# aristoteleo/spateo-release

Hardware: AMD Instinct MI355X
Metric: cells/s per SparseVFC EM iter (higher is better)
Workload: dtype f32

## Files before the change

### spateo-release_amd/csrc/mvf_common.h

```cpp
#pragma once
#include <hip/hip_runtime.h>

#include <cmath>
#include <cstdarg>
#include <cstdint>
#include <cstdio>
#include <cstdlib>
#include <algorithm>

#include "../../include/mvf.h"

namespace mvf {

char* err_buf();
int set_error(const char* fmt, ...);
enum DebugOpt { DBG_CONK_FORM = 0, DBG_SLICE_LEN, DBG_SOLVE_SMALL_OFF, DBG_LR_TIMING, DBG_LR_NO_DEFLATE, DBG_DEFL_BLOCK, DBG_DEFL_APPS, DBG_LR_NO_DIRECT, DBG_DIRECT_ACCEPT, DBG_COUNT };
long long debug_opt(DebugOpt which);
int device_cu_count();

#define MVF_CHECK_HIP(expr)                                                                      \
    do {                                                                                         \
        hipError_t _e = (expr);                                                                  \
        if (_e != hipSuccess) return ::mvf::set_error("%s failed: %s", #expr, hipGetErrorString(_e)); \
    } while (0)

#define MVF_REQUIRE(cond, ...)                       \
    do {                                             \
        if (!(cond)) return ::mvf::set_error(__VA_ARGS__); \
    } while (0)

#define MVF_LAUNCH_CHECK() MVF_CHECK_HIP(hipGetLastError())

constexpr int WAVE = 64;

constexpr double LOG2E = 1.4426950408889634074;

template <typename T>
struct Vec4;
template <>
struct Vec4<float> {
    using type = float4;
};
template <>
struct Vec4<double> {
    using type = double4;
};

__device__ __forceinline__ float exp2_neg(float e) { return __builtin_amdgcn_exp2f(e); }
__device__ __forceinline__ double exp2_neg(double e) { return exp2(e); }

template <typename T>
__device__ __forceinline__ T kernel_value(T px, T py, T pz, T cx, T cy, T cz) {
    const T dx = px - cx, dy = py - cy, dz = pz - cz;
    const T e = fma(dz, dz, fma(dy, dy, dx * dx));
    return exp2_neg(-e);
}

template <int D, typename T>
__device__ __forceinline__ T kernel_value_d(const T (&p)[D], const T (&c)[D]) {
    T e = T(0);
#pragma unroll
    for (int k = 0; k < D; ++k) {
        const T t = p[k] - c[k];
        e = fma(t, t, e);
    }
    return exp2_neg(-e);
}

__device__ __forceinline__ double wave_sum(double v) {
#pragma unroll
    for (int o = 32; o > 0; o >>= 1) v += __shfl_down(v, o, 64);
    return v;
}
__device__ __forceinline__ double wave_min(double v) {
#pragma unroll
    for (int o = 32; o > 0; o >>= 1) v = fmin(v, __shfl_down(v, o, 64));
    return v;
}

template <int NT>
__device__ __forceinline__ double block_sum(double v, double* sm ) {
    v = wave_sum(v);
    const int lane = threadIdx.x & 63, w = threadIdx.x >> 6;
    __syncthreads();
    if (lane == 0) sm[w] = v;
    __syncthreads();
    double t = 0.0;
    if (threadIdx.x == 0) {
#pragma unroll
        for (int i = 0; i < NT / 64; ++i) t += sm[i];
    }
    return t;
}
template <int NT>
__device__ __forceinline__ double block_min(double v, double* sm) {
    v = wave_min(v);
    const int lane = threadIdx.x & 63, w = threadIdx.x >> 6;
    __syncthreads();
    if (lane == 0) sm[w] = v;
    __syncthreads();
    double t = INFINITY;
    if (threadIdx.x == 0) {
#pragma unroll
        for (int i = 0; i < NT / 64; ++i) t = fmin(t, sm[i]);
    }
    return t;
}

struct EvalAffine {
    double alpha[3], jmul;
    double A[9];
    double b[3];
};

inline EvalAffine eval_affine_from_host(const double* affine) {
    EvalAffine af;
    af.alpha[0] = af.alpha[1] = af.alpha[2] = 1.0, af.jmul = 1.0;
    for (int i = 0; i < 9; ++i) af.A[i] = 0.0;
    for (int i = 0; i < 3; ++i) af.b[i] = 0.0;
    if (affine) {
        for (int i = 0; i < 3; ++i) af.alpha[i] = affine[i];
        af.jmul = affine[3];
        for (int i = 0; i < 9; ++i) af.A[i] = affine[4 + i];
        for (int i = 0; i < 3; ++i) af.b[i] = affine[13 + i];
    }
    return af;
}

inline int64_t cdiv(int64_t a, int64_t b) { return (a + b - 1) / b; }
inline size_t align_up(size_t x, size_t a) { return (x + a - 1) / a * a; }

}
```

### spateo-release_amd/csrc/mvf_em.hip

```cpp
#include "mvf_common.h"

namespace mvf {

constexpr int APPLY_CHUNK = 512;

template <typename T, int CPT>
__global__ __launch_bounds__(256) void apply_kernel(const T* __restrict__ x4, int64_t n, const T* __restrict__ ctrl4,
                                                    int64_t m, T s, const double* __restrict__ C ,
                                                    T* __restrict__ V4, const T* __restrict__ y4,
                                                    const T* __restrict__ P, T* __restrict__ r,
                                                    double* __restrict__ block_pr) {
    using V4T = typename Vec4<T>::type;
    __shared__ __attribute__((aligned(16))) unsigned char smem_raw[APPLY_CHUNK * (sizeof(V4T) + 4 * sizeof(double))];
    V4T* sc = reinterpret_cast<V4T*>(smem_raw);
    double4* sC = reinterpret_cast<double4*>(smem_raw + APPLY_CHUNK * sizeof(V4T));

    const int64_t base = ((int64_t)blockIdx.x * 256) * CPT + threadIdx.x;
    T px[CPT], py[CPT], pz[CPT];
    double v0[CPT], v1[CPT], v2[CPT];
#pragma unroll
    for (int c = 0; c < CPT; ++c) {
        const int64_t i = base + (int64_t)c * 256;
        V4T xv = (i < n) ? reinterpret_cast<const V4T*>(x4)[i] : V4T{0, 0, 0, 0};
        px[c] = xv.x * s;
        py[c] = xv.y * s;
        pz[c] = xv.z * s;
        v0[c] = v1[c] = v2[c] = 0.0;
    }

    for (int64_t m0 = 0; m0 < m; m0 += APPLY_CHUNK) {
        const int mc = (int)min((int64_t)APPLY_CHUNK, m - m0);
        __syncthreads();
        for (int j = threadIdx.x; j < APPLY_CHUNK; j += 256) {
            if (j < mc) {
                V4T cv = reinterpret_cast<const V4T*>(ctrl4)[m0 + j];
                sc[j] = V4T{cv.x * s, cv.y * s, cv.z * s, 0};
                const double* cp = C + (m0 + j) * 3;
                sC[j] = double4{cp[0], cp[1], cp[2], 0.0};
            } else {
                sc[j] = V4T{0, 0, 0, 0};
                sC[j] = double4{0.0, 0.0, 0.0, 0.0};
            }
        }
        __syncthreads();
        const int mc_pad = (mc + 3) & ~3;
#pragma unroll 4
        for (int j = 0; j < mc_pad; ++j) {
            const V4T cv = sc[j];
            const double4 cc = sC[j];
#pragma unroll
            for (int c = 0; c < CPT; ++c) {
                const double k = (double)kernel_value(px[c], py[c], pz[c], cv.x, cv.y, cv.z);
                v0[c] = fma(k, cc.x, v0[c]);
                v1[c] = fma(k, cc.y, v1[c]);
                v2[c] = fma(k, cc.z, v2[c]);
            }
        }
    }

    double pr = 0.0;
#pragma unroll
    for (int c = 0; c < CPT; ++c) {
        const int64_t i = base + (int64_t)c * 256;
        if (i < n) {
            reinterpret_cast<V4T*>(V4)[i] = V4T{(T)v0[c], (T)v1[c], (T)v2[c], 0};
            if (y4) {
                const V4T yv = reinterpret_cast<const V4T*>(y4)[i];
                const double d0 = (double)yv.x - (double)(T)v0[c], d1 = (double)yv.y - (double)(T)v1[c],
                             d2 = (double)yv.z - (double)(T)v2[c];
                const double rr = d0 * d0 + d1 * d1 + d2 * d2;
                r[i] = (T)rr;
                if (P) pr += (double)P[i] * (double)(T)rr;
            }
        }
    }
    if (y4 && P && block_pr) {
        __shared__ double red[4];
        const double t = block_sum<256>(pr, red);
        if (threadIdx.x == 0) block_pr[blockIdx.x] = t;
    }
}

__global__ __launch_bounds__(256) void sum_partials_kernel(const double* __restrict__ partials, int64_t nb, int stride,
                                                           int K, double* __restrict__ out, int overwrite = 0) {
    __shared__ double red[4];
    for (int k = 0; k < K; ++k) {
        double s = 0.0;
        for (int64_t b = threadIdx.x; b < nb; b += 256) s += partials[b * stride + k];
        const double t = block_sum<256>(s, red);
        if (threadIdx.x == 0) out[k] = overwrite ? t : out[k] + t;
        __syncthreads();
    }
}

template <typename T>
__global__ __launch_bounds__(256) void estep_min_kernel(const T* __restrict__ r, int64_t n, double inv2s2,
                                                        double* __restrict__ block_min_out,
                                                        double* __restrict__ block_zero_out) {
    double mn = INFINITY, zeros = 0.0;
    for (int64_t i = (int64_t)blockIdx.x * 256 + threadIdx.x; i < n; i += (int64_t)gridDim.x * 256) {
        const double t1 = exp(-(double)r[i] * inv2s2);
        if (t1 == 0.0)
            zeros += 1.0;
        else
            mn = fmin(mn, t1);
    }
    __shared__ double red[4];
    const double bm = block_min<256>(mn, red);
    const double bz = block_sum<256>(zeros, red);
    if (threadIdx.x == 0) {
        block_min_out[blockIdx.x] = bm;
        block_zero_out[blockIdx.x] = bz;
    }
}

__global__ __launch_bounds__(256) void estep_min_finish(const double* __restrict__ bmin, const double* __restrict__ bzero,
                                                        int nb, double* __restrict__ mins) {
    double mn = INFINITY, z = 0.0;
    for (int i = threadIdx.x; i < nb; i += 256) {
        mn = fmin(mn, bmin[i]);
        z += bzero[i];
    }
    __shared__ double red[4];
    const double a = block_min<256>(mn, red);
    const double b = block_sum<256>(z, red);
    if (threadIdx.x == 0) {
        mins[0] = a;
        mins[1] = b;
    }
}

template <typename T>
__global__ __launch_bounds__(256) void estep_p_kernel(const T* __restrict__ r, int64_t n, double inv2s2, double t2,
                                                      double minP, double theta, double zero_fill_host,
                                                      const double* __restrict__ fill_dev, T* __restrict__ Pout,
                                                      double* __restrict__ block_stats) {
    double zero_fill = zero_fill_host;
    if (fill_dev) {
        const double f = *fill_dev;
        zero_fill = (f < INFINITY) ? f : 0.0;
    }
    double s_pr = 0.0, s_p = 0.0, s_pf = 0.0, s_cnt = 0.0, s_zero = 0.0;
    for (int64_t i = (int64_t)blockIdx.x * 256 + threadIdx.x; i < n; i += (int64_t)gridDim.x * 256) {
        const double ri = (double)r[i];
        double t1 = exp(-ri * inv2s2);
        if (t1 == 0.0) {
            t1 = zero_fill;
            s_zero += 1.0;
        }
        const double p = t1 / (t1 + t2);
        s_pr += p * ri;
        s_p += p;
        const T pf = (T)fmax(p, minP);
        Pout[i] = pf;
        s_pf += (double)pf;
        s_cnt += ((double)pf > theta) ? 1.0 : 0.0;
    }
    __shared__ double red[4];
    const double a = block_sum<256>(s_pr, red);
    const double b = block_sum<256>(s_p, red);
    const double c = block_sum<256>(s_pf, red);
    const double d = block_sum<256>(s_cnt, red);
    const double e = block_sum<256>(s_zero, red);
    if (threadIdx.x == 0) {
        double* o = block_stats + (int64_t)blockIdx.x * 5;
        o[0] = a, o[1] = b, o[2] = c, o[3] = d, o[4] = e;
    }
}

__global__ __launch_bounds__(256) void quadform_kernel(const double* __restrict__ K, const double* __restrict__ C,
                                                       int64_t m, int nrhs, double* __restrict__ row_out) {
    const int64_t i = blockIdx.x;
    double acc = 0.0;
    for (int d = 0; d < nrhs; ++d) {
        double t = 0.0;
        for (int64_t j = threadIdx.x; j < m; j += 256) t += K[i * m + j] * C[j * nrhs + d];
        acc += t * C[i * nrhs + d];
    }
    __shared__ double red[4];
    const double s = block_sum<256>(acc, red);
    if (threadIdx.x == 0) row_out[i] = s;
}

__device__ __forceinline__ int64_t tri_offset(int64_t i, int64_t m) { return i * m - i * (i - 1) / 2; }

__global__ __launch_bounds__(256) void sym_pack_kernel(const double* __restrict__ G, int64_t m, double* __restrict__ tri) {
    const int64_t i = blockIdx.y;
    const int64_t j = (int64_t)blockIdx.x * 256 + threadIdx.x;
    if (j < m && j >= i) tri[tri_offset(i, m) + (j - i)] = G[i * m + j];
}

__global__ __launch_bounds__(256) void sym_unpack_kernel(const double* __restrict__ tri, int64_t m, double* __restrict__ G) {
    const int64_t i = blockIdx.y;
    const int64_t j = (int64_t)blockIdx.x * 256 + threadIdx.x;
    if (j >= m) return;
    G[i * m + j] = j >= i ? tri[tri_offset(i, m) + (j - i)] : tri[tri_offset(j, m) + (i - j)];
}

}

using namespace mvf;

extern "C" int mvf_sym_pack(const double* G, int64_t m, double* tri, void* stream) {
    MVF_REQUIRE(m >= 0 && m <= 65535, "mvf_sym_pack: bad m");
    if (m == 0) return 0;
// ... 167 lines not shown
```

### spateo-release_amd/csrc/mvf_gram.hip

```cpp
#include "mvf_common.h"
#include <type_traits>

namespace mvf {

constexpr int GT = 128;
constexpr int GCHUNK = 256;

typedef double f64x4 __attribute__((ext_vector_type(4)));

struct GramPlan {
    int nt = 0, npairs = 0;
    int njobs = 0, edge2 = 0;
    int64_t slice_len = 0, nslices = 0;
    int64_t phase_slices = 0, nphases = 1;
    int64_t rslice_len = 0, rslices = 0;
    int rcolblocks = 0;
    size_t gram_bytes = 0, rhs_bytes = 0;
};

constexpr int RHS_CPT = 2;
constexpr int RHS_COLS = 256 * RHS_CPT;

static int gram_slots() { return 2 * device_cu_count(); }

// ... 88 lines not shown
        const int64_t ib = (int64_t)tj * GT + wj * 64 + a * 16 + (lane & 15);
        if (ia < m) {
            const V4 c = ctrl4[ia];
            ax[a] = c.x * s, ay[a] = c.y * s, az[a] = c.z * s;
        } else {
            ax[a] = ay[a] = az[a] = PAD;
        }
        if (ib < m) {
            const V4 c = ctrl4[ib];
            bx[a] = c.x * s, by[a] = c.y * s, bz[a] = c.z * s;
        } else {
            bx[a] = by[a] = bz[a] = PAD;
        }
    }

    f64x4 acc[4][4];
#pragma unroll
    for (int a = 0; a < 4; ++a)
#pragma unroll
        for (int b = 0; b < 4; ++b) acc[a][b] = f64x4{0.0, 0.0, 0.0, 0.0};

    auto load_cell = [&](int64_t i) -> V4 {
        if (i < n1) {
            const V4 xv = x4[i];
            return V4{xv.x * s, xv.y * s, xv.z * s, P[i]};
        }
        return V4{0, 0, 0, 0};
    };

    const int nchunks = (int)((n1 - n0 + GCHUNK - 1) / GCHUNK);
    V4 stage = load_cell(n0 + tid);
    cells[0][tid] = stage;
    const int quarter = lane >> 4;

    for (int c = 0; c < nchunks; ++c) {
        __syncthreads();
        if (c + 1 < nchunks) stage = load_cell(n0 + (int64_t)(c + 1) * GCHUNK + tid);
        const V4* cb = cells[c & 1];
#pragma unroll 2
        for (int st = 0; st < GCHUNK / 4; ++st) {
            const V4 cell = cb[4 * st + quarter];
            double fa[4], fb[4];
#pragma unroll
            for (int a = 0; a < 4; ++a) {
                fa[a] = (double)kernel_value(cell.x, cell.y, cell.z, ax[a], ay[a], az[a]) * (double)cell.w;
                fb[a] = (double)kernel_value(cell.x, cell.y, cell.z, bx[a], by[a], bz[a]);
            }
#ifdef MVF_PROBE_SETPRIO_RECOMPUTE
            __builtin_amdgcn_s_setprio(1);
#endif
#pragma unroll
            for (int a = 0; a < 4; ++a)
#pragma unroll
                for (int b = 0; b < 4; ++b)
                    acc[a][b] = __builtin_amdgcn_mfma_f64_16x16x4f64(fa[a], fb[b], acc[a][b], 0, 0, 0);
#ifdef MVF_PROBE_SETPRIO_RECOMPUTE
            __builtin_amdgcn_s_setprio(0);
#endif
        }
        if (c + 1 < nchunks) cells[(c + 1) & 1][tid] = stage;
    }

    double* out = partial + ((size_t)slice * npairs + pair) * (size_t)(GT * GT);
#pragma unroll
    for (int a = 0; a < 4; ++a)
#pragma unroll
        for (int b = 0; b < 4; ++b)
#pragma unroll
            for (int r = 0; r < 4; ++r) {
                const int row = wi * 64 + a * 16 + quarter + 4 * r;
                const int col = wj * 64 + b * 16 + (lane & 15);
                out[row * GT + col] = acc[a][b][r];
            }
}

constexpr int UB = 16;

template <typename T>
__global__ __launch_bounds__(256) void ublk_build_kernel(const typename Vec4<T>::type* __restrict__ x4, int64_t n,
                                                         int64_t n_pad, const typename Vec4<T>::type* __restrict__ ctrl4,
                                                         int64_t m, int64_t m_pad, T s, int cb_per_block,
                                                         T* __restrict__ ublk) {
    using V4 = typename Vec4<T>::type;
    extern __shared__ __attribute__((aligned(16))) unsigned char ublk_smem[];
    V4* sctrl = reinterpret_cast<V4*>(ublk_smem);
    const int64_t cb0 = (int64_t)blockIdx.y * cb_per_block;
    const int ncb = (int)min((int64_t)cb_per_block, m_pad / UB - cb0);
    for (int j = threadIdx.x; j < ncb * UB; j += 256) {
        const int64_t c = cb0 * UB + j;
        if (c < m) {
            const V4 cv = ctrl4[c];
            sctrl[j] = V4{cv.x * s, cv.y * s, cv.z * s, 1};
        } else {
            sctrl[j] = V4{0, 0, 0, 0};
        }
    }
    __syncthreads();
    constexpr int PER = 16 / sizeof(T);
    constexpr int Q = UB / PER;
    constexpr int LPC = UB / PER;
    typedef T vec_t __attribute__((ext_vector_type(PER)));
    const int lane = threadIdx.x & 63;
    const int64_t wbase = (int64_t)blockIdx.x * 256 + (threadIdx.x & ~63);
    if (wbase >= n_pad) return;
    const int j0 = (lane % LPC) * PER;
    T px[Q], py[Q], pz[Q];
    bool live[Q];
#pragma unroll
    for (int q = 0; q < Q; ++q) {
        const int64_t i = wbase + (64 / LPC) * q + lane / LPC;
        live[q] = i < n;
        px[q] = py[q] = pz[q] = T(0);
        if (live[q]) {
            const V4 xv = x4[i];
            px[q] = xv.x * s, py[q] = xv.y * s, pz[q] = xv.z * s;
        }
    }
    for (int b = 0; b < ncb; ++b) {
        V4 cv[PER];
#pragma unroll
        for (int jj = 0; jj < PER; ++jj) cv[jj] = sctrl[b * UB + j0 + jj];
        vec_t* dst = reinterpret_cast<vec_t*>(ublk + ((cb0 + b) * n_pad + wbase) * UB) + lane;
#pragma unroll
        for (int q = 0; q < Q; ++q) {
            vec_t o;
#pragma unroll
            for (int jj = 0; jj < PER; ++jj) {
                const T k = kernel_value(px[q], py[q], pz[q], cv[jj].x, cv[jj].y, cv[jj].z);
                o[jj] = (live[q] && cv[jj].w != 0) ? k : T(0);
            }
            __builtin_nontemporal_store(o, dst + 64 * q);
        }
    }
}

#ifndef MVF_UG
#define MVF_UG 2
#endif
constexpr int UG = MVF_UG;

#ifndef MVF_CACHED_WPS
#define MVF_CACHED_WPS 2
#endif
#ifndef MVF_DBL_UG
#define MVF_DBL_UG 1
#endif
#ifndef MVF_DBL_NBUF
#define MVF_DBL_NBUF 2
#endif
template <typename T> struct CachedPipe { static constexpr int UGT = UG, NBUF = 2; };
template <> struct CachedPipe<double> { static constexpr int UGT = MVF_DBL_UG, NBUF = MVF_DBL_NBUF; };

template <typename T, int NA, int NB, bool TRI, int DW = -1, bool PAIR2 = false>
__device__ __forceinline__ void cached_block(const T* __restrict__ ublk, const T* __restrict__ P, int64_t n,
                                             int64_t n_pad, int64_t n0, int64_t n1, int64_t rb0, int64_t cb0,
                                             double* __restrict__ out, int orow0, int ocol0, int64_t rb1 = 0,
                                             double* __restrict__ out1 = nullptr) {
    constexpr int UGT = CachedPipe<T>::UGT, NBUF = CachedPipe<T>::NBUF;
    static_assert(DW < 0 || (NA == 2 && NB == 8 && !TRI && DW < 4), "balanced diagonal shape is a sub-shape of 2 x 8");
    static_assert(!PAIR2 || (NA == 4 && NB == 4 && !TRI && DW < 0), "paired edge shape: 2 + 2 row blocks x 4 column blocks");
    const int lane = threadIdx.x & 63;
    const int li = lane & 15, lk = lane >> 4;
    auto blk_live = [](int a, int b) constexpr {
        if (DW >= 0) return b >= (a == 0 ? DW : 7 - DW);
        return !TRI || b >= a;
    };
    auto rblk = [](int a) constexpr { return DW >= 0 ? (a == 0 ? DW : 7 - DW) : a; };

    const T* pa[NA];
    const T* pb[NB];
#pragma unroll
    for (int a = 0; a < NA; ++a)
        pa[a] = ublk + ((PAIR2 ? (a < 2 ? rb0 + a : rb1 + (a - 2)) : rb0 + rblk(a)) * n_pad + n0 + lk) * UB + li;
#pragma unroll
    for (int b = 0; b < NB; ++b) pb[b] = ublk + ((cb0 + b) * n_pad + n0 + lk) * UB + li;

    f64x4 acc[NA][NB];
#pragma unroll
    for (int a = 0; a < NA; ++a)
#pragma unroll
        for (int b = 0; b < NB; ++b) acc[a][b] = f64x4{0.0, 0.0, 0.0, 0.0};

    T ua[NBUF][UGT][NA], ub[NBUF][UGT][NB], pp[NBUF][UGT];
    const int ngroups = (int)((n1 - n0) / (4 * UGT));

    constexpr int SUPER = 4096 / (UGT * 4 * UB * (int)sizeof(T));
    const T* pP = P + n0 + lk;
    const int pmax = (int)min((int64_t)0x3fffffff, n - 1 - n0 - lk);
    auto load_group = [&](int64_t gbase, int s, bool in_tail, T(&A)[UGT][NA], T(&B)[UGT][NB], T(&Pq)[UGT]) {
#pragma unroll
        for (int q = 0; q < UGT; ++q) {
            const int64_t off = (gbase * UGT) * (4 * UB) + (s * UGT + q) * (4 * UB);
#ifdef MVF_PROBE_NO_LOAD
#pragma unroll
            for (int a = 0; a < NA; ++a) A[q][a] = (T)(0.5 + lane * 1e-3 + off * 1e-9);
#pragma unroll
            for (int b = 0; b < NB; ++b) B[q][b] = (T)(0.25 + lane * 1e-3);
#else
#pragma unroll
            for (int a = 0; a < NA; ++a) A[q][a] = pa[a][off];
#pragma unroll
            for (int b = 0; b < NB; ++b) B[q][b] = pb[b][off];
#endif
#if defined(MVF_PROBE_NO_LOAD) || defined(MVF_PROBE_NO_P)
            Pq[q] = T(1);
#else
            const int64_t poff = (gbase * UGT) * 4 + (s * UGT + q) * 4;
            Pq[q] = in_tail ? pP[min((int)poff, pmax)] : pP[poff];
#endif
        }
    };
    auto compute_group = [&](const T(&A)[UGT][NA], const T(&B)[UGT][NB], const T(&Pq)[UGT]) {
#pragma unroll
        for (int q = 0; q < UGT; ++q) {
            double fa[NA], fb[NB];
            const double pd = (double)Pq[q];
#pragma unroll
            for (int a = 0; a < NA; ++a) {
#ifdef MVF_PROBE_NO_P
                fa[a] = (double)A[q][a];
#else
                fa[a] = (double)A[q][a] * pd;
#endif
            }
#pragma unroll
            for (int b = 0; b < NB; ++b) fb[b] = (double)B[q][b];
#ifdef MVF_PROBE_NO_MFMA
#pragma unroll
            for (int a = 0; a < NA; ++a) acc[a][a][0] += fa[a] + fb[a];
#else
#ifndef MVF_PROBE_NO_SETPRIO
            __builtin_amdgcn_s_setprio(1);
#endif
#pragma unroll
            for (int a = 0; a < NA; ++a)
#pragma unroll
                for (int b = 0; b < NB; ++b)
                    if (blk_live(a, b))
                        acc[a][b] = __builtin_amdgcn_mfma_f64_16x16x4f64(fa[a], fb[b], acc[a][b], 0, 0, 0);
#ifndef MVF_PROBE_NO_SETPRIO
            __builtin_amdgcn_s_setprio(0);
#endif
#endif
        }
    };

    static_assert(SUPER % NBUF == 0, "ring slots must be static inside a superblock");
    constexpr int AHEAD = NBUF - 1;
    const int64_t live = max((int64_t)0, min(n1, n) - n0);
    const int ng_main = (int)(min((int64_t)ngroups, live / (4 * UGT)) / SUPER) * SUPER;
#pragma unroll
    for (int s = 0; s < AHEAD; ++s)
        if (s < ng_main) load_group(0, s, false, ua[s], ub[s], pp[s]);
    for (int g0 = 0; g0 < ng_main; g0 += SUPER) {
#pragma unroll
        for (int s = 0; s < SUPER; ++s) {
            if (g0 + s + AHEAD < ng_main)
                load_group(g0, s + AHEAD, false, ua[(s + AHEAD) % NBUF], ub[(s + AHEAD) % NBUF], pp[(s + AHEAD) % NBUF]);
            compute_group(ua[s % NBUF], ub[s % NBUF], pp[s % NBUF]);
            __builtin_amdgcn_sched_barrier(0);
        }
    }
    for (int g = ng_main; g < ngroups; ++g) {
        load_group(g, 0, true, ua[0], ub[0], pp[0]);
        compute_group(ua[0], ub[0], pp[0]);
    }

#pragma unroll
    for (int a = 0; a < NA; ++a)
#pragma unroll
        for (int b = 0; b < NB; ++b)
            if (blk_live(a, b)) {
#pragma unroll
                for (int r = 0; r < 4; ++r) {
                    const int row = orow0 + (PAIR2 ? (a & 1) : rblk(a)) * 16 + lk + 4 * r;
                    const int col = ocol0 + b * 16 + li;
                    double* o = (PAIR2 && a >= 2) ? out1 : out;
                    __builtin_nontemporal_store(acc[a][b][r], &o[row * GT + col]);
                }
            }
}

template <typename T>
__global__ __launch_bounds__(256, MVF_CACHED_WPS) void gram_cached_kernel(const T* __restrict__ ublk, const T* __restrict__ P,
                                                             int64_t n, int64_t n_pad, int64_t m, int nt, int npairs,
                                                             int64_t slice_len, int64_t slice0,
                                                             double* __restrict__ partial, int njobs, int edge2) {
    constexpr int TB = GT / UB;
    const int wave = __builtin_amdgcn_readfirstlane(threadIdx.x >> 6);
    int ti, tj, pair;
    int64_t slice;
    if constexpr (sizeof(T) == 4) {
        pair = blockIdx.x % npairs;
        slice = blockIdx.x / npairs;
        decode_pair(pair, nt, ti, tj);
    } else {
        const int job = blockIdx.x % njobs;
        slice = blockIdx.x / njobs;
        if (edge2 && job >= npairs - nt) {
            const int e = job - (npairs - nt);
            ti = 2 * e, tj = nt - 1;
            if (ti + 1 < nt) {
                const int64_t n0p = (slice0 + slice) * slice_len;
                const int64_t n1p = min(n_pad, n0p + slice_len);
                auto slot = [&](int t) { return t * nt - t * (t - 1) / 2 + (tj - t); };
                double* oa = partial + ((size_t)slice * npairs + slot(ti)) * (size_t)(GT * GT);
                double* ob = partial + ((size_t)slice * npairs + slot(ti + 1)) * (size_t)(GT * GT);
                cached_block<T, 4, 4, false, -1, true>(ublk, P, n, n_pad, n0p, n1p, (int64_t)ti * TB + 2 * wave,
                                                       (int64_t)tj * TB, oa, 32 * wave, 0, (int64_t)(ti + 1) * TB + 2 * wave, ob);
                return;
            }
        } else if (edge2) {
            decode_pair(job, nt - 1, ti, tj);
        } else {
            decode_pair(job, nt, ti, tj);
        }
        pair = ti * nt - ti * (ti - 1) / 2 + (tj - ti);
    }
    const int64_t n0 = (slice0 + slice) * slice_len;
    const int64_t n1 = min(n_pad, n0 + slice_len);
    double* out = partial + ((size_t)slice * npairs + pair) * (size_t)(GT * GT);
    const int64_t rb = (int64_t)ti * TB, cb = (int64_t)tj * TB;
#ifdef MVF_PROBE_NO_SKIP
    constexpr bool skip = false;
#else
    constexpr bool skip = sizeof(T) == 4;
#endif
#ifndef MVF_PROBE_F64_SHAPES
#define MVF_PROBE_F64_SHAPES 0
#endif
    constexpr bool use_edge = skip || (MVF_PROBE_F64_SHAPES & 1);
    constexpr bool use_diag = skip || (MVF_PROBE_F64_SHAPES & 2);
    if (ti != tj || !use_diag) {
        const int64_t live_cols = m - (int64_t)tj * GT;
        if (use_edge && ti != tj && live_cols <= 4 * UB)
            cached_block<T, 2, 4, false>(ublk, P, n, n_pad, n0, n1, rb + 2 * wave, cb, out, 32 * wave, 0);
        else
            cached_block<T, 2, 8, false>(ublk, P, n, n_pad, n0, n1, rb + 2 * wave, cb, out, 32 * wave, 0);
    } else {
        switch (wave) {
            case 0: cached_block<T, 2, 8, false, 0>(ublk, P, n, n_pad, n0, n1, rb, cb, out, 0, 0); break;
            case 1: cached_block<T, 2, 8, false, 1>(ublk, P, n, n_pad, n0, n1, rb, cb, out, 0, 0); break;
            case 2: cached_block<T, 2, 8, false, 2>(ublk, P, n, n_pad, n0, n1, rb, cb, out, 0, 0); break;
            default: cached_block<T, 2, 8, false, 3>(ublk, P, n, n_pad, n0, n1, rb, cb, out, 0, 0); break;
        }
    }
}

template <typename T>
__global__ __launch_bounds__(256) void rhs_kernel(const T* __restrict__ x4, const T* __restrict__ P,
                                                  const T* __restrict__ y4, int64_t n, const T* __restrict__ ctrl4,
                                                  int64_t m, T s, int64_t slice_len, double* __restrict__ rpart) {
    using V4T = typename Vec4<T>::type;
    __shared__ V4T sx[GCHUNK];
    __shared__ V4T sw[GCHUNK];
    const int64_t slice = blockIdx.y;
    const int64_t n0 = slice * slice_len, n1 = min(n, n0 + slice_len);
    T cx[RHS_CPT], cy[RHS_CPT], cz[RHS_CPT];
    double r0[RHS_CPT], r1[RHS_CPT], r2[RHS_CPT];
#pragma unroll
    for (int c = 0; c < RHS_CPT; ++c) {
        const int64_t j = (int64_t)blockIdx.x * RHS_COLS + c * 256 + threadIdx.x;
        if (j < m) {
            const V4T cv = reinterpret_cast<const V4T*>(ctrl4)[j];
            cx[c] = cv.x * s, cy[c] = cv.y * s, cz[c] = cv.z * s;
        } else {
            cx[c] = cy[c] = cz[c] = T(0);
        }
        r0[c] = r1[c] = r2[c] = 0.0;
    }
    for (int64_t c0 = n0; c0 < n1; c0 += GCHUNK) {
        __syncthreads();
        const int64_t i = c0 + threadIdx.x;
        if (i < n1) {
            const V4T xv = reinterpret_cast<const V4T*>(x4)[i];
            const V4T yv = reinterpret_cast<const V4T*>(y4)[i];
            const T p = P[i];
            sx[threadIdx.x] = V4T{xv.x * s, xv.y * s, xv.z * s, 0};
            sw[threadIdx.x] = V4T{yv.x * p, yv.y * p, yv.z * p, 0};
        } else {
            sx[threadIdx.x] = V4T{0, 0, 0, 0};
            sw[threadIdx.x] = V4T{0, 0, 0, 0};
        }
        __syncthreads();
#pragma unroll 4
        for (int q = 0; q < GCHUNK; ++q) {
            const V4T xv = sx[q];
            const V4T wv = sw[q];
#pragma unroll
            for (int c = 0; c < RHS_CPT; ++c) {
                const double k = (double)kernel_value(xv.x, xv.y, xv.z, cx[c], cy[c], cz[c]);
                r0[c] = fma(k, (double)wv.x, r0[c]);
                r1[c] = fma(k, (double)wv.y, r1[c]);
                r2[c] = fma(k, (double)wv.z, r2[c]);
            }
        }
    }
#pragma unroll
    for (int c = 0; c < RHS_CPT; ++c) {
        const int64_t j = (int64_t)blockIdx.x * RHS_COLS + c * 256 + threadIdx.x;
        if (j < m) {
            double4* o = reinterpret_cast<double4*>(rpart + ((size_t)slice * m + j) * 4);
            *o = double4{r0[c], r1[c], r2[c], 0.0};
        }
    }
}

__global__ __launch_bounds__(256) void gram_reduce_kernel(const double* __restrict__ partial, int64_t nslices, int nt,
                                                          int npairs, int64_t m, double* __restrict__ G, int accumulate) {
    const int pair = blockIdx.y;
    int ti, tj;
    decode_pair(pair, nt, ti, tj);
    const int e = blockIdx.x * 256 + threadIdx.x;
    const int row = e / GT, col = e % GT;
    const int64_t i = (int64_t)ti * GT + row, j = (int64_t)tj * GT + col;
    if (i >= m || j >= m) return;
    if (ti == tj && col < row) return;
    const double* p = partial + (size_t)pair * (GT * GT) + e;
    const size_t stride = (size_t)npairs * (GT * GT);
    double a[8] = {0.0, 0.0, 0.0, 0.0, 0.0, 0.0, 0.0, 0.0};
    int64_t s = 0;
    for (; s + 8 <= nslices; s += 8) {
#pragma unroll
        for (int q = 0; q < 8; ++q) a[q] += p[(s + q) * stride];
    }
    for (int q = 0; s < nslices; ++s, ++q) a[q] += p[s * stride];
    double acc = ((a[0] + a[1]) + (a[2] + a[3])) + ((a[4] + a[5]) + (a[6] + a[7]));
    if (accumulate) acc += G[i * m + j];
    G[i * m + j] = acc;
    if (i != j) G[j * m + i] = acc;
}

__global__ __launch_bounds__(256) void rhs_reduce_kernel(const double* __restrict__ rpart, int64_t rslices, int64_t m,
                                                         double* __restrict__ R ) {
    __shared__ double sm[16][16][3];
    const int tx = threadIdx.x & 15, ty = threadIdx.x >> 4;
    const int64_t j = (int64_t)blockIdx.x * 16 + tx;
    double a0 = 0.0, a1 = 0.0, a2 = 0.0;
    if (j < m) {
        for (int64_t s = ty; s < rslices; s += 16) {
            const double4 v = *reinterpret_cast<const double4*>(rpart + ((size_t)s * m + j) * 4);
            a0 += v.x, a1 += v.y, a2 += v.z;
        }
    }
    sm[ty][tx][0] = a0, sm[ty][tx][1] = a1, sm[ty][tx][2] = a2;
    __syncthreads();
    if (threadIdx.x < 48) {
        const int o = threadIdx.x / 3, comp = threadIdx.x % 3;
        const int64_t jo = (int64_t)blockIdx.x * 16 + o;
        double t = 0.0;
#pragma unroll
        for (int q = 0; q < 16; ++q) t += sm[q][o][comp];
        if (jo < m) R[jo * 3 + comp] = t;
    }
}

}

using namespace mvf;

extern "C" size_t mvf_gram_workspace_bytes(int64_t n, int64_t m, mvf_dtype dtype) {
    if (n <= 0 || m <= 0) return 0;
    const GramPlan p = make_plan(n, m, dtype);
    return align_up(p.gram_bytes, 256) + align_up(p.rhs_bytes, 256);
}

extern "C" int mvf_gram_stages(int stages, const void* x4, const void* P, const void* y4, int64_t n,
                               const void* ctrl4, int64_t m, double beta, double* G, double* R, void* workspace,
                               size_t workspace_bytes, mvf_dtype dtype, void* stream) {
    MVF_REQUIRE(n >= 0 && m >= 0, "mvf_gram: bad shape");
    MVF_REQUIRE(beta >= 0.0 && std::isfinite(beta), "mvf_gram: beta must be finite and >= 0");
    MVF_REQUIRE(dtype == MVF_F32 || dtype == MVF_F64, "mvf_gram: bad dtype %d", (int)dtype);
    MVF_REQUIRE(stages > 0 && stages <= 15, "mvf_gram: bad stage mask %d", stages);
    if (m == 0) return 0;
    MVF_REQUIRE(!(stages & MVF_GRAM_STAGE_REDUCE) || G, "mvf_gram: null G");
    MVF_REQUIRE(!(stages & MVF_GRAM_STAGE_REDUCE_RHS) || R, "mvf_gram: null R");
    hipStream_t st = (hipStream_t)stream;
    if (n == 0) {
        if (stages & MVF_GRAM_STAGE_REDUCE) MVF_CHECK_HIP(hipMemsetAsync(G, 0, sizeof(double) * m * m, st));
        if (stages & MVF_GRAM_STAGE_REDUCE_RHS) MVF_CHECK_HIP(hipMemsetAsync(R, 0, sizeof(double) * m * 3, st));
        return 0;
    }
    MVF_REQUIRE(x4 && P && ctrl4, "mvf_gram: null input");
    MVF_REQUIRE(!(stages & MVF_GRAM_STAGE_RHS) || y4, "mvf_gram: null y4");
    const GramPlan p = make_plan(n, m, dtype);
    const size_t need = align_up(p.gram_bytes, 256) + align_up(p.rhs_bytes, 256);
    MVF_REQUIRE(workspace && workspace_bytes >= need, "mvf_gram: workspace too small (%zu < %zu)", workspace_bytes, need);
    MVF_REQUIRE((int64_t)p.phase_slices * p.npairs < (1LL << 31), "mvf_gram: too many jobs");
    MVF_REQUIRE(p.rslices <= 65535, "mvf_gram: rhs slice count too large");
    double* gpart = (double*)workspace;
    double* rpart = (double*)((char*)workspace + align_up(p.gram_bytes, 256));
    const double s = std::sqrt(beta * LOG2E);
    dim3 rgrid((unsigned)p.rcolblocks, (unsigned)p.rslices);
    if (stages & MVF_GRAM_STAGE_TILES) {
        MVF_REQUIRE(p.nphases == 1 || G, "mvf_gram: null G (the tile stage reduces all but its last phase)");
        for (int64_t ph = 0; ph < p.nphases; ++ph) {
            const int64_t s0 = ph * p.phase_slices, ns = std::min(p.phase_slices, p.nslices - s0);
            const unsigned njobs = (unsigned)(ns * p.npairs);
            if (dtype == MVF_F32)
                hipLaunchKernelGGL(gram_f64acc_kernel<float>, dim3(njobs), dim3(256), 0, st, (const float4*)x4,
                                   (const float*)P, n, (const float4*)ctrl4, m, (float)s, p.nt, p.npairs, p.slice_len, s0,
                                   gpart);
            else
                hipLaunchKernelGGL(gram_f64acc_kernel<double>, dim3(njobs), dim3(256), 0, st, (const double4*)x4,
                                   (const double*)P, n, (const double4*)ctrl4, m, s, p.nt, p.npairs, p.slice_len, s0,
                                   gpart);
            if (ph + 1 < p.nphases)
                hipLaunchKernelGGL(gram_reduce_kernel, dim3(GT * GT / 256, (unsigned)p.npairs), dim3(256), 0, st, gpart,
                                   ns, p.nt, p.npairs, m, G, ph > 0 ? 1 : 0);
        }
        MVF_LAUNCH_CHECK();
    }
    if (stages & MVF_GRAM_STAGE_RHS) {
        if (dtype == MVF_F32)
            hipLaunchKernelGGL(rhs_kernel<float>, rgrid, dim3(256), 0, st, (const float*)x4, (const float*)P,
                               (const float*)y4, n, (const float*)ctrl4, m, (float)s, p.rslice_len, rpart);
        else
            hipLaunchKernelGGL(rhs_kernel<double>, rgrid, dim3(256), 0, st, (const double*)x4, (const double*)P,
                               (const double*)y4, n, (const double*)ctrl4, m, s, p.rslice_len, rpart);
        MVF_LAUNCH_CHECK();
    }
    if (stages & MVF_GRAM_STAGE_REDUCE) {
        const int64_t s0 = (p.nphases - 1) * p.phase_slices;
        hipLaunchKernelGGL(gram_reduce_kernel, dim3(GT * GT / 256, (unsigned)p.npairs), dim3(256), 0, st, gpart,
                           p.nslices - s0, p.nt, p.npairs, m, G, p.nphases > 1 ? 1 : 0);
        MVF_LAUNCH_CHECK();
    }
    if (stages & MVF_GRAM_STAGE_REDUCE_RHS) {
        hipLaunchKernelGGL(rhs_reduce_kernel, dim3((unsigned)cdiv(m, 16)), dim3(256), 0, st, rpart, p.rslices, m, R);
        MVF_LAUNCH_CHECK();
    }
    return 0;
}

static inline int64_t ublk_npad(int64_t n) { return cdiv(n, GCHUNK) * GCHUNK; }
static inline int64_t ublk_mpad(int64_t m) { return cdiv(m, GT) * GT; }

extern "C" size_t mvf_ublk_bytes(int64_t n, int64_t m, mvf_dtype dtype) {
    if (n <= 0 || m <= 0) return 0;
    return (size_t)ublk_npad(n) * (size_t)ublk_mpad(m) * (dtype == MVF_F64 ? sizeof(double) : sizeof(float));
}

extern "C" int mvf_ublk_build(const void* x4, int64_t n, const void* ctrl4, int64_t m, double beta, void* ublk,
                              size_t ublk_bytes, mvf_dtype dtype, void* stream) {
    MVF_REQUIRE(n > 0 && m > 0, "mvf_ublk_build: need n > 0 and m > 0");
    MVF_REQUIRE(dtype == MVF_F32 || dtype == MVF_F64, "mvf_ublk_build: bad dtype %d", (int)dtype);
    MVF_REQUIRE(beta >= 0.0 && std::isfinite(beta), "mvf_ublk_build: beta must be finite and >= 0");
    MVF_REQUIRE(x4 && ctrl4 && ublk, "mvf_ublk_build: null pointer");
    MVF_REQUIRE(ublk_bytes >= mvf_ublk_bytes(n, m, dtype), "mvf_ublk_build: buffer too small (%zu < %zu)", ublk_bytes,
                mvf_ublk_bytes(n, m, dtype));
    hipStream_t st = (hipStream_t)stream;
    const int64_t n_pad = ublk_npad(n), m_pad = ublk_mpad(m);
    const int cb_per_block = 32;
    dim3 grid((unsigned)(n_pad / 256), (unsigned)cdiv(m_pad / UB, cb_per_block));
    MVF_REQUIRE(grid.y <= 65535, "mvf_ublk_build: m too large");
    const double s = std::sqrt(beta * LOG2E);
    if (dtype == MVF_F32)
        hipLaunchKernelGGL(ublk_build_kernel<float>, grid, dim3(256), cb_per_block * UB * sizeof(float4), st,
                           (const float4*)x4, n, n_pad, (const float4*)ctrl4, m, m_pad, (float)s, cb_per_block,
                           (float*)ublk);
    else
        hipLaunchKernelGGL(ublk_build_kernel<double>, grid, dim3(256), cb_per_block * UB * sizeof(double4), st,
                           (const double4*)x4, n, n_pad, (const double4*)ctrl4, m, m_pad, s, cb_per_block,
                           (double*)ublk);
    MVF_LAUNCH_CHECK();
    return 0;
}

extern "C" int mvf_gram_cached(int stages, const void* ublk, const void* x4, const void* P, const void* y4, int64_t n,
                               const void* ctrl4, int64_t m, double beta, double* G, double* R, void* workspace,
                               size_t workspace_bytes, mvf_dtype dtype, void* stream) {
    MVF_REQUIRE(n > 0 && m > 0, "mvf_gram_cached: need n > 0 and m > 0");
    MVF_REQUIRE(dtype == MVF_F32 || dtype == MVF_F64, "mvf_gram_cached: bad dtype %d", (int)dtype);
    MVF_REQUIRE(stages > 0 && stages <= 15, "mvf_gram_cached: bad stage mask %d", stages);
    MVF_REQUIRE(ublk && P, "mvf_gram_cached: null pointer");
    hipStream_t st = (hipStream_t)stream;
    if (stages & MVF_GRAM_STAGE_TILES) {
        const GramPlan p = make_plan(n, m, dtype);
        const size_t need = align_up(p.gram_bytes, 256) + align_up(p.rhs_bytes, 256);
        MVF_REQUIRE(workspace && workspace_bytes >= need, "mvf_gram_cached: workspace too small (%zu < %zu)",
                    workspace_bytes, need);
        MVF_REQUIRE((int64_t)p.phase_slices * p.npairs < (1LL << 31), "mvf_gram_cached: too many jobs");
        MVF_REQUIRE(p.nphases == 1 || G, "mvf_gram_cached: null G (the tile stage reduces all but its last phase)");
        for (int64_t ph = 0; ph < p.nphases; ++ph) {
            const int64_t s0 = ph * p.phase_slices, ns = std::min(p.phase_slices, p.nslices - s0);
            const unsigned njobs = (unsigned)(ns * p.npairs);
            if (dtype == MVF_F32)
                hipLaunchKernelGGL(gram_cached_kernel<float>, dim3(njobs), dim3(256), 0, st, (const float*)ublk,
                                   (const float*)P, n, ublk_npad(n), m, p.nt, p.npairs, p.slice_len, s0,
                                   (double*)workspace, p.npairs, 0);
            else
                hipLaunchKernelGGL(gram_cached_kernel<double>, dim3((unsigned)(ns * p.njobs)), dim3(256), 0, st,
                                   (const double*)ublk, (const double*)P, n, ublk_npad(n), m, p.nt, p.npairs, p.slice_len, s0,
                                   (double*)workspace, p.njobs, p.edge2);
            if (ph + 1 < p.nphases)
                hipLaunchKernelGGL(gram_reduce_kernel, dim3(GT * GT / 256, (unsigned)p.npairs), dim3(256), 0, st,
                                   (const double*)workspace, ns, p.nt, p.npairs, m, G, ph > 0 ? 1 : 0);
        }
        MVF_LAUNCH_CHECK();
    }
    const int rest = stages & (MVF_GRAM_STAGE_RHS | MVF_GRAM_STAGE_REDUCE | MVF_GRAM_STAGE_REDUCE_RHS);
    if (rest)
        return mvf_gram_stages(rest, x4, P, y4, n, ctrl4, m, beta, G, R, workspace, workspace_bytes, dtype, stream);
    return 0;
}

extern "C" int mvf_gram(const void* x4, const void* P, const void* y4, int64_t n, const void* ctrl4, int64_t m,
                        double beta, double* G, double* R, void* workspace, size_t workspace_bytes, mvf_dtype dtype,
                        void* stream) {
    return mvf_gram_stages(MVF_GRAM_STAGE_TILES | MVF_GRAM_STAGE_RHS | MVF_GRAM_STAGE_REDUCE | MVF_GRAM_STAGE_REDUCE_RHS, x4,
                           P, y4, n, ctrl4, m,
                           beta, G, R, workspace, workspace_bytes, dtype, stream);
}
```

Measured before the change: 7.387 million.

## Pack kernel exp pairs, use buffer loads and pre-widened P in Gram

Computes the Gaussian kernel distance for two cells at once with packed f32x2 FMA in the apply and RHS kernels. In the cached Gram kernel it switches f32 operand loads to raw buffer loads with scalar offsets. It also feeds a P vector pre-widened to double, produced by a new widen kernel each phase in extra workspace. RHS weights are stored as doubles in shared memory to avoid per-iteration conversions. The costs are an extra kernel launch, more workspace and more shared memory.

```diff
diff --git a/spateo-release_amd/csrc/mvf_common.h b/spateo-release_amd/csrc/mvf_common.h
--- a/spateo-release_amd/csrc/mvf_common.h
+++ b/spateo-release_amd/csrc/mvf_common.h
@@ -54,6 +54,13 @@
     const T dx = px - cx, dy = py - cy, dz = pz - cz;
     const T e = fma(dz, dz, fma(dy, dy, dx * dx));
     return exp2_neg(-e);
+}
+
+typedef float f32x2 __attribute__((ext_vector_type(2)));
+__device__ __forceinline__ f32x2 kernel_value_pk(f32x2 px, f32x2 py, f32x2 pz, f32x2 cx, f32x2 cy, f32x2 cz) {
+    const f32x2 dx = px - cx, dy = py - cy, dz = pz - cz;
+    const f32x2 e = __builtin_elementwise_fma(dz, dz, __builtin_elementwise_fma(dy, dy, dx * dx));
+    return f32x2{exp2_neg(-e.x), exp2_neg(-e.y)};
 }
 
 template <int D, typename T>
diff --git a/spateo-release_amd/csrc/mvf_em.hip b/spateo-release_amd/csrc/mvf_em.hip
--- a/spateo-release_amd/csrc/mvf_em.hip
+++ b/spateo-release_amd/csrc/mvf_em.hip
@@ -1,4 +1,5 @@
 #include "mvf_common.h"
+#include <type_traits>
 
 namespace mvf {
 
@@ -48,9 +49,21 @@
         for (int j = 0; j < mc_pad; ++j) {
             const V4T cv = sc[j];
             const double4 cc = sC[j];
+            T kv[CPT];
+            if constexpr (std::is_same<T, float>::value && CPT >= 2) {
+#pragma unroll
+                for (int c = 0; c < CPT; c += 2) {
+                    const f32x2 k2 = kernel_value_pk(f32x2{px[c], px[c + 1]}, f32x2{py[c], py[c + 1]}, f32x2{pz[c], pz[c + 1]},
+                                                     f32x2{cv.x, cv.x}, f32x2{cv.y, cv.y}, f32x2{cv.z, cv.z});
+                    kv[c] = k2.x, kv[c + 1] = k2.y;
+                }
+            } else {
+#pragma unroll
+                for (int c = 0; c < CPT; ++c) kv[c] = kernel_value(px[c], py[c], pz[c], cv.x, cv.y, cv.z);
+            }
 #pragma unroll
             for (int c = 0; c < CPT; ++c) {
-                const double k = (double)kernel_value(px[c], py[c], pz[c], cv.x, cv.y, cv.z);
+                const double k = (double)kv[c];
                 v0[c] = fma(k, cc.x, v0[c]);
                 v1[c] = fma(k, cc.y, v1[c]);
                 v2[c] = fma(k, cc.z, v2[c]);
diff --git a/spateo-release_amd/csrc/mvf_gram.hip b/spateo-release_amd/csrc/mvf_gram.hip
--- a/spateo-release_amd/csrc/mvf_gram.hip
+++ b/spateo-release_amd/csrc/mvf_gram.hip
@@ -264,7 +264,7 @@
 template <> struct CachedPipe<double> { static constexpr int UGT = MVF_DBL_UG, NBUF = MVF_DBL_NBUF; };
 
 template <typename T, int NA, int NB, bool TRI, int DW = -1, bool PAIR2 = false>
-__device__ __forceinline__ void cached_block(const T* __restrict__ ublk, const T* __restrict__ P, int64_t n,
+__device__ __forceinline__ void cached_block(const T* __restrict__ ublk, const double* __restrict__ P, int64_t n,
                                              int64_t n_pad, int64_t n0, int64_t n1, int64_t rb0, int64_t cb0,
                                              double* __restrict__ out, int orow0, int ocol0, int64_t rb1 = 0,
                                              double* __restrict__ out1 = nullptr) {
@@ -287,19 +287,35 @@
 #pragma unroll
     for (int b = 0; b < NB; ++b) pb[b] = ublk + ((cb0 + b) * n_pad + n0 + lk) * UB + li;
 
+    constexpr bool BUF = sizeof(T) == 4;
+    constexpr int BUF_RSRC_WORD3 = 0x00020000;
+    __amdgpu_buffer_rsrc_t ra[NA], rbuf[NB];
+    const int voff = (lk * UB + li) * (int)sizeof(T);
+    if constexpr (BUF) {
+        const int nbytes = (int)((n1 - n0) * UB * (int64_t)sizeof(T));
+#pragma unroll
+        for (int a = 0; a < NA; ++a)
+            ra[a] = __builtin_amdgcn_make_buffer_rsrc(
+                (void*)(ublk + ((PAIR2 ? (a < 2 ? rb0 + a : rb1 + (a - 2)) : rb0 + rblk(a)) * n_pad + n0) * UB), (short)0, nbytes,
+                BUF_RSRC_WORD3);
+#pragma unroll
+        for (int b = 0; b < NB; ++b)
+            rbuf[b] = __builtin_amdgcn_make_buffer_rsrc((void*)(ublk + ((cb0 + b) * n_pad + n0) * UB), (short)0, nbytes, BUF_RSRC_WORD3);
+    }
     f64x4 acc[NA][NB];
 #pragma unroll
     for (int a = 0; a < NA; ++a)
 #pragma unroll
         for (int b = 0; b < NB; ++b) acc[a][b] = f64x4{0.0, 0.0, 0.0, 0.0};
 
-    T ua[NBUF][UGT][NA], ub[NBUF][UGT][NB], pp[NBUF][UGT];
+    T ua[NBUF][UGT][NA], ub[NBUF][UGT][NB];
+    double pp[NBUF][UGT];
     const int ngroups = (int)((n1 - n0) / (4 * UGT));
 
     constexpr int SUPER = 4096 / (UGT * 4 * UB * (int)sizeof(T));
-    const T* pP = P + n0 + lk;
+    const double* pP = P + n0 + lk;
     const int pmax = (int)min((int64_t)0x3fffffff, n - 1 - n0 - lk);
-    auto load_group = [&](int64_t gbase, int s, bool in_tail, T(&A)[UGT][NA], T(&B)[UGT][NB], T(&Pq)[UGT]) {
+    auto load_group = [&](int64_t gbase, int s, bool in_tail, T(&A)[UGT][NA], T(&B)[UGT][NB], double(&Pq)[UGT]) {
 #pragma unroll
         for (int q = 0; q < UGT; ++q) {
             const int64_t off = (gbase * UGT) * (4 * UB) + (s * UGT + q) * (4 * UB);
@@ -309,24 +325,35 @@
 #pragma unroll
             for (int b = 0; b < NB; ++b) B[q][b] = (T)(0.25 + lane * 1e-3);
 #else
+            if constexpr (BUF) {
+                const int soff = __builtin_amdgcn_readfirstlane((int)(gbase * UGT) * (4 * UB) * (int)sizeof(T));
+                const int imm = (s * UGT + q) * (4 * UB) * (int)sizeof(T);
+#pragma unroll
+                for (int a = 0; a < NA; ++a)
+                    A[q][a] = __builtin_bit_cast(T, (int)__builtin_amdgcn_raw_buffer_load_b32(ra[a], voff + imm, soff, 0));
+#pragma unroll
+                for (int b = 0; b < NB; ++b)
+                    B[q][b] = __builtin_bit_cast(T, (int)__builtin_amdgcn_raw_buffer_load_b32(rbuf[b], voff + imm, soff, 0));
+            } else {
 #pragma unroll
             for (int a = 0; a < NA; ++a) A[q][a] = pa[a][off];
 #pragma unroll
             for (int b = 0; b < NB; ++b) B[q][b] = pb[b][off];
+            }
 #endif
 #if defined(MVF_PROBE_NO_LOAD) || defined(MVF_PROBE_NO_P)
-            Pq[q] = T(1);
+            Pq[q] = 1.0;
 #else
             const int64_t poff = (gbase * UGT) * 4 + (s * UGT + q) * 4;
             Pq[q] = in_tail ? pP[min((int)poff, pmax)] : pP[poff];
 #endif
         }
     };
-    auto compute_group = [&](const T(&A)[UGT][NA], const T(&B)[UGT][NB], const T(&Pq)[UGT]) {
+    auto compute_group = [&](const T(&A)[UGT][NA], const T(&B)[UGT][NB], const double(&Pq)[UGT]) {
 #pragma unroll
         for (int q = 0; q < UGT; ++q) {
             double fa[NA], fb[NB];
-            const double pd = (double)Pq[q];
+            const double pd = Pq[q];
 #pragma unroll
             for (int a = 0; a < NA; ++a) {
 #ifdef MVF_PROBE_NO_P
@@ -394,7 +421,7 @@
 }
 
 template <typename T>
-__global__ __launch_bounds__(256, MVF_CACHED_WPS) void gram_cached_kernel(const T* __restrict__ ublk, const T* __restrict__ P,
+__global__ __launch_bounds__(256, MVF_CACHED_WPS) void gram_cached_kernel(const T* __restrict__ ublk, const double* __restrict__ P,
                                                              int64_t n, int64_t n_pad, int64_t m, int nt, int npairs,
                                                              int64_t slice_len, int64_t slice0,
                                                              double* __restrict__ partial, int njobs, int edge2) {
@@ -459,13 +486,19 @@
     }
 }
 
+__global__ __launch_bounds__(256) void widen_p_kernel(const float* __restrict__ P, int64_t n, int64_t c0, int64_t c1,
+                                                      double* __restrict__ Pd) {
+    const int64_t i = c0 + (int64_t)blockIdx.x * 256 + threadIdx.x;
+    if (i < c1) Pd[i - c0] = i < n ? (double)P[i] : 0.0;
+}
+
 template <typename T>
 __global__ __launch_bounds__(256) void rhs_kernel(const T* __restrict__ x4, const T* __restrict__ P,
                                                   const T* __restrict__ y4, int64_t n, const T* __restrict__ ctrl4,
                                                   int64_t m, T s, int64_t slice_len, double* __restrict__ rpart) {
     using V4T = typename Vec4<T>::type;
     __shared__ V4T sx[GCHUNK];
-    __shared__ V4T sw[GCHUNK];
+    __shared__ double4 sw[GCHUNK];
     const int64_t slice = blockIdx.y;
     const int64_t n0 = slice * slice_len, n1 = min(n, n0 + slice_len);
     T cx[RHS_CPT], cy[RHS_CPT], cz[RHS_CPT];
@@ -489,22 +522,32 @@
             const V4T yv = reinterpret_cast<const V4T*>(y4)[i];
             const T p = P[i];
             sx[threadIdx.x] = V4T{xv.x * s, xv.y * s, xv.z * s, 0};
-            sw[threadIdx.x] = V4T{yv.x * p, yv.y * p, yv.z * p, 0};
+            sw[threadIdx.x] = double4{(double)(T)(yv.x * p), (double)(T)(yv.y * p), (double)(T)(yv.z * p), 0.0};
         } else {
             sx[threadIdx.x] = V4T{0, 0, 0, 0};
-            sw[threadIdx.x] = V4T{0, 0, 0, 0};
+            sw[threadIdx.x] = double4{0.0, 0.0, 0.0, 0.0};
         }
         __syncthreads();
 #pragma unroll 4
         for (int q = 0; q < GCHUNK; ++q) {
             const V4T xv = sx[q];
-            const V4T wv = sw[q];
+            const double4 wv = sw[q];
+            T kv[RHS_CPT];
+            if constexpr (std::is_same<T, float>::value) {
+                static_assert(RHS_CPT == 2, "one packed pair per cell");
+                const f32x2 k2 = kernel_value_pk(f32x2{xv.x, xv.x}, f32x2{xv.y, xv.y}, f32x2{xv.z, xv.z},
+                                                 f32x2{cx[0], cx[1]}, f32x2{cy[0], cy[1]}, f32x2{cz[0], cz[1]});
+                kv[0] = k2.x, kv[1] = k2.y;
+            } else {
+#pragma unroll
+                for (int c = 0; c < RHS_CPT; ++c) kv[c] = kernel_value(xv.x, xv.y, xv.z, cx[c], cy[c], cz[c]);
+            }
 #pragma unroll
             for (int c = 0; c < RHS_CPT; ++c) {
-                const double k = (double)kernel_value(xv.x, xv.y, xv.z, cx[c], cy[c], cz[c]);
-                r0[c] = fma(k, (double)wv.x, r0[c]);
-                r1[c] = fma(k, (double)wv.y, r1[c]);
-                r2[c] = fma(k, (double)wv.z, r2[c]);
+                const double k = (double)kv[c];
+                r0[c] = fma(k, wv.x, r0[c]);
+                r1[c] = fma(k, wv.y, r1[c]);
+                r2[c] = fma(k, wv.z, r2[c]);
             }
         }
     }
@@ -571,10 +614,17 @@
 
 using namespace mvf;
 
+static inline int64_t ublk_npad(int64_t n) { return cdiv(n, GCHUNK) * GCHUNK; }
+static inline int64_t ublk_mpad(int64_t m) { return cdiv(m, GT) * GT; }
+static inline int64_t phase_cells(const GramPlan& p, int64_t n) { return std::min(ublk_npad(n), p.phase_slices * p.slice_len); }
+static inline size_t widened_p_bytes(const GramPlan& p, int64_t n, mvf_dtype dtype) {
+    return dtype == MVF_F32 ? align_up(sizeof(double) * (size_t)phase_cells(p, n), 256) : 0;
+}
+
 extern "C" size_t mvf_gram_workspace_bytes(int64_t n, int64_t m, mvf_dtype dtype) {
     if (n <= 0 || m <= 0) return 0;
     const GramPlan p = make_plan(n, m, dtype);
-    return align_up(p.gram_bytes, 256) + align_up(p.rhs_bytes, 256);
+    return align_up(p.gram_bytes, 256) + align_up(p.rhs_bytes, 256) + widened_p_bytes(p, n, dtype);
 }
 
 extern "C" int mvf_gram_stages(int stages, const void* x4, const void* P, const void* y4, int64_t n,
@@ -645,9 +695,6 @@
     return 0;
 }
 
-static inline int64_t ublk_npad(int64_t n) { return cdiv(n, GCHUNK) * GCHUNK; }
-static inline int64_t ublk_mpad(int64_t m) { return cdiv(m, GT) * GT; }
-
 extern "C" size_t mvf_ublk_bytes(int64_t n, int64_t m, mvf_dtype dtype) {
     if (n <= 0 || m <= 0) return 0;
     return (size_t)ublk_npad(n) * (size_t)ublk_mpad(m) * (dtype == MVF_F64 ? sizeof(double) : sizeof(float));
@@ -689,21 +736,30 @@
     hipStream_t st = (hipStream_t)stream;
     if (stages & MVF_GRAM_STAGE_TILES) {
         const GramPlan p = make_plan(n, m, dtype);
-        const size_t need = align_up(p.gram_bytes, 256) + align_up(p.rhs_bytes, 256);
+        const size_t pd_off = align_up(p.gram_bytes, 256) + align_up(p.rhs_bytes, 256);
+        const size_t need = pd_off + widened_p_bytes(p, n, dtype);
         MVF_REQUIRE(workspace && workspace_bytes >= need, "mvf_gram_cached: workspace too small (%zu < %zu)",
                     workspace_bytes, need);
+        const int64_t n_pad = ublk_npad(n);
+        double* const pd = (double*)((char*)workspace + pd_off);
         MVF_REQUIRE((int64_t)p.phase_slices * p.npairs < (1LL << 31), "mvf_gram_cached: too many jobs");
+        MVF_REQUIRE(dtype != MVF_F32 || p.slice_len * UB * (int64_t)sizeof(float) < (1LL << 31),
+                    "mvf_gram_cached: slice too long");
         MVF_REQUIRE(p.nphases == 1 || G, "mvf_gram_cached: null G (the tile stage reduces all but its last phase)");
         for (int64_t ph = 0; ph < p.nphases; ++ph) {
             const int64_t s0 = ph * p.phase_slices, ns = std::min(p.phase_slices, p.nslices - s0);
             const unsigned njobs = (unsigned)(ns * p.npairs);
-            if (dtype == MVF_F32)
+            if (dtype == MVF_F32) {
+                const int64_t c0 = s0 * p.slice_len, c1 = std::min(n_pad, c0 + ns * p.slice_len);
+                hipLaunchKernelGGL(widen_p_kernel, dim3((unsigned)((c1 - c0) / 256)), dim3(256), 0, st, (const float*)P, n,
+                                   c0, c1, pd);
+                const double* Pd = (const double*)((uintptr_t)pd - (uintptr_t)c0 * sizeof(double));
                 hipLaunchKernelGGL(gram_cached_kernel<float>, dim3(njobs), dim3(256), 0, st, (const float*)ublk,
-                                   (const float*)P, n, ublk_npad(n), m, p.nt, p.npairs, p.slice_len, s0,
+                                   Pd, n, n_pad, m, p.nt, p.npairs, p.slice_len, s0,
                                    (double*)workspace, p.npairs, 0);
-            else
+            } else
                 hipLaunchKernelGGL(gram_cached_kernel<double>, dim3((unsigned)(ns * p.njobs)), dim3(256), 0, st,
-                                   (const double*)ublk, (const double*)P, n, ublk_npad(n), m, p.nt, p.npairs, p.slice_len, s0,
+                                   (const double*)ublk, (const double*)P, n, n_pad, m, p.nt, p.npairs, p.slice_len, s0,
                                    (double*)workspace, p.njobs, p.edge2);
             if (ph + 1 < p.nphases)
                 hipLaunchKernelGGL(gram_reduce_kernel, dim3(GT * GT / 256, (unsigned)p.npairs), dim3(256), 0, st,
```

Measured after the change: 7.513 million (median of 6 runs). 1.02x the previous value.
